# skhu101/SHERF

Measured on AMD Instinct MI355X. Metric: rendered rays/sec at 512x512x64 samples (ImportanceRenderer.forward), higher is better.
Workload: dtype f16 MFMA (fp16 operands rounded to nearest, one product, fp32 accumulate), fp32 elsewhere

## Files before the change

sherf_amd/csrc/gather.hip:

```cpp
#include "common.h"

#ifndef SHERF_GATHER_BRANCHLESS
#define SHERF_GATHER_BRANCHLESS 0
#endif

namespace {

struct Levels { sherf_vox_level l[3]; };

__device__ __forceinline__ void axpy4(float4& a, float w, const float4 v) {
    a.x += w * v.x; a.y += w * v.y; a.z += w * v.z; a.w += w * v.w;
}

__device__ __forceinline__ float clampf(float x, float lo, float hi) { return fminf(fmaxf(x, lo), hi); }

typedef _Float16 h16x4 __attribute__((ext_vector_type(4)));
template <bool HT>
__device__ __forceinline__ float4 ldq(const void* __restrict__ base, size_t idx) {
    if constexpr (HT) {
        const h16x4 v = reinterpret_cast<const h16x4*>(base)[idx];
        return make_float4((float)v[0], (float)v[1], (float)v[2], (float)v[3]);
    } else {
        return reinterpret_cast<const float4*>(base)[idx];
    }
// ... 115 lines not shown
                    }
                    if constexpr (BL) {
#pragma unroll
                    for (int t = 0; t < 8; ++t) {
                        const float w = rec[t].x ? ((t & 1) ? fx : 1.f - fx) * (((t >> 1) & 1) ? fy : 1.f - fy) * ((t >> 2) ? fz : 1.f - fz) : 0.f;
                        const size_t r = (size_t)(rec[t].x ? rec[t].y : 0u) * 24;
                        axpy4(acc[0], w, ldq<HT>(lev.rows, r + l));
                        axpy4(acc[1], w, ldq<HT>(lev.rows, r + 8 + l));
                        axpy4(acc[2], w, ldq<HT>(lev.rows, r + 16 + l));
                    }
                    } else {
#pragma unroll
                    for (int t = 0; t < 8; ++t) {
                        if (rec[t].x) {
                            const float w = ((t & 1) ? fx : 1.f - fx) * (((t >> 1) & 1) ? fy : 1.f - fy) * ((t >> 2) ? fz : 1.f - fz);
                            const size_t r = (size_t)rec[t].y * 24;
                            axpy4(acc[0], w, ldq<HT>(lev.rows, r + l));
                            axpy4(acc[1], w, ldq<HT>(lev.rows, r + 8 + l));
                            axpy4(acc[2], w, ldq<HT>(lev.rows, r + 16 + l));
                        }
                    }
                    }
                }
            }
        } else {
            acc[0] = acc[1] = acc[2] = make_float4(0.f, 0.f, 0.f, 0.f);
            if (mode != 2) {
                extras[(tile * 12 + l) * 32 + j] = 0.f;
                if (l < 4) extras[(tile * 12 + 8 + l) * 32 + j] = 0.f;
            }
        }
        if (mode == 2) {
            if (c < nv)
#pragma unroll
                for (int s = 0; s < 3; ++s) {
                    float4 t = tokens[((tile * 3 + s) * 8 + l) * 32 + j];
                    t.x += acc[s].x; t.y += acc[s].y; t.z += acc[s].z; t.w += acc[s].w;
                    tokens[((tile * 3 + s) * 8 + l) * 32 + j] = t;
                }
            continue;
        }
#pragma unroll
        for (int s = 0; s < 3; ++s) tokens[((tile * 3 + s) * 8 + l) * 32 + j] = acc[s];
    }
}

typedef _Float16 h16x8 __attribute__((ext_vector_type(8)));
constexpr int kPeStride = 120;
__device__ __forceinline__ int64_t banded_first_pair(int b, int g, int64_t n_pairs, int dbg) {
    const bool banded = !(dbg & 1024) && g % 8 == 0;
    if (!banded) return b;
    const int64_t per_xcd = (n_pairs + 7) / 8;
    return (int64_t)(b / 8) < per_xcd ? (int64_t)(b % 8) * per_xcd + b / 8 : n_pairs;
}
struct f8 { float4 a, b; };
__device__ __forceinline__ void axpy8(f8& acc, float w, const void* __restrict__ base, uint32_t idx8) {
    const h16x8 v = *reinterpret_cast<const h16x8*>(static_cast<const char*>(base) + (size_t)(idx8 * 16u));
    acc.a.x += w * (float)v[0]; acc.a.y += w * (float)v[1]; acc.a.z += w * (float)v[2]; acc.a.w += w * (float)v[3];
    acc.b.x += w * (float)v[4]; acc.b.y += w * (float)v[5]; acc.b.z += w * (float)v[6]; acc.b.w += w * (float)v[7];
}

template <bool STAGE, bool PE = false, bool PF = false>
__global__ void __launch_bounds__(256) gather_tokens_h8_kernel(const int32_t* __restrict__ counters, const float* __restrict__ geom,
                                                               const void* __restrict__ planes_f, int P, const void* __restrict__ feat_f,
                                                               int Hf, int Wf, const float4* __restrict__ img4, int H, int W, Levels lv,
                                                               const float4* __restrict__ tok_bias, const float* __restrict__ bounds,
                                                               const float* __restrict__ vox_min, int3 vox_sh, int64_t capacity,
                                                               float4* __restrict__ tokens, float* __restrict__ extras, int dbg, int mode,
                                                               uint4* __restrict__ pefrag) {
    const int64_t nv = min((int64_t)counters[0], capacity);
    int64_t t_lo, t_hi;
    sherf_part_range((nv + 31) / 32, (mode >> 8) & 255, (mode >> 16) & 255, t_lo, t_hi);
    mode &= 255;
    const int64_t n_tiles = t_hi - t_lo, n_pairs = (n_tiles + 1) / 2;
    extern __shared__ __attribute__((aligned(16))) uint2 s_wp[];
    int s_n1 = 0;
    if constexpr (STAGE) {
        const int n1 = (lv.l[1].D * lv.l[1].H * lv.l[1].W + 31) / 32, n2 = (lv.l[2].D * lv.l[2].H * lv.l[2].W + 31) / 32;
        s_n1 = n1;
        if ((banded_first_pair(blockIdx.x, gridDim.x, n_pairs, dbg)) < n_pairs && mode != 1) {
            for (int i = threadIdx.x; i < n1; i += 256) s_wp[i] = reinterpret_cast<const uint2*>(lv.l[1].wp)[i];
            for (int i = threadIdx.x; i < n2; i += 256) s_wp[n1 + i] = reinterpret_cast<const uint2*>(lv.l[2].wp)[i];
        }
        __syncthreads();
    }
    const int l = threadIdx.x & 3;
    const int js = threadIdx.x >> 2;
    const bool banded = !(dbg & 1024) && gridDim.x % 8 == 0;
    const int64_t per_xcd = (n_pairs + 7) / 8, slots = gridDim.x / 8;
    for (int64_t it = banded ? blockIdx.x / 8 : blockIdx.x; it < (banded ? per_xcd : n_pairs); it += banded ? slots : gridDim.x) {
        const int64_t pair = banded ? (int64_t)(blockIdx.x % 8) * per_xcd + it : it;
        if (pair >= n_pairs) break;
        int64_t tile = pair * 2 + (js >> 5);
        const int j = js & 31;
        if (tile >= n_tiles) continue;
        tile += t_lo;
        const int64_t c = tile * 32 + j;
        f8 acc[3];
        if (mode == 2) { for (int s_ = 0; s_ < 3; ++s_) acc[s_].a = acc[s_].b = make_float4(0.f, 0.f, 0.f, 0.f); }
        else { for (int s_ = 0; s_ < 3; ++s_) { acc[s_].a = tok_bias[8 * s_ + 2 * l]; acc[s_].b = tok_bias[8 * s_ + 2 * l + 1]; } }
        float4 rgb = make_float4(0.f, 0.f, 0.f, 0.f);
        const bool valid = c < nv;
        float xv[3] = {0.f, 0.f, 0.f};
        if (valid) {
            const float* gm = geom + c * 8;
            const float xc[3] = {gm[0], gm[1], gm[2]};
            xv[0] = xc[0]; xv[1] = xc[1]; xv[2] = xc[2];
            if (mode != 2) {
                if (l < 3) { extras[(tile * 12 + 2 * l) * 32 + j] = gm[2 * l]; extras[(tile * 12 + 2 * l + 1) * 32 + j] = gm[2 * l + 1]; }
            }
            float n[3];
#pragma unroll
            for (int a = 0; a < 3; ++a) n[a] = 2.f * (xc[a] - bounds[a]) / (bounds[3 + a] - bounds[a]) - 1.f;
#pragma unroll
            for (int p = 0; p < 3; ++p) {
                if ((dbg & 8) || mode == 2) break;
                const float ga = p == 2 ? n[2] : n[0];
                const float gb = p == 1 ? n[2] : n[1];
                float px = clampf(((ga + 1.f) * P - 1.f) * 0.5f, -2.f, (float)P + 1.f);
                float py = clampf(((gb + 1.f) * P - 1.f) * 0.5f, -2.f, (float)P + 1.f);
                float x0 = floorf(px), y0 = floorf(py), fx = px - x0, fy = py - y0;
                int xi = (int)x0, yi = (int)y0;
#pragma unroll
                for (int dy = 0; dy < 2; ++dy)
#pragma unroll
                    for (int dx = 0; dx < 2; ++dx) {
                        int xx = xi + dx, yy = yi + dy;
                        if (xx >= 0 && xx < P && yy >= 0 && yy < P)
                            axpy8(acc[p], (dx ? fx : 1.f - fx) * (dy ? fy : 1.f - fy), planes_f, (uint32_t)(((p * P + yy) * P + xx) * 4 + l));
                    }
            }
            if (!(dbg & 16) && mode != 2) {
                float gx = 2.0f * gm[6] / (float)W - 1.0f, gy = 2.0f * gm[7] / (float)H - 1.0f;
                float px = clampf((gx + 1.f) * 0.5f * (Wf - 1), -2.f, (float)Wf + 1.f);
                float py = clampf((gy + 1.f) * 0.5f * (Hf - 1), -2.f, (float)Hf + 1.f);
                float x0 = floorf(px), y0 = floorf(py), fx = px - x0, fy = py - y0;
                int xi = (int)x0, yi = (int)y0;
#pragma unroll
                for (int dy = 0; dy < 2; ++dy)
#pragma unroll
                    for (int dx = 0; dx < 2; ++dx) {
                        int xx = xi + dx, yy = yi + dy;
                        if (xx >= 0 && xx < Wf && yy >= 0 && yy < Hf) {
                            const float w = (dx ? fx : 1.f - fx) * (dy ? fy : 1.f - fy);
                            const uint32_t t = (uint32_t)((yy * Wf + xx) * 8);
                            axpy8(acc[0], w, feat_f, t + l);
                            axpy8(acc[1], w, feat_f, t + 4 + l);
                        }
                    }
                px = clampf((gx + 1.f) * 0.5f * (W - 1), -2.f, (float)W + 1.f);
                py = clampf((gy + 1.f) * 0.5f * (H - 1), -2.f, (float)H + 1.f);
                x0 = floorf(px); y0 = floorf(py); fx = px - x0; fy = py - y0;
                xi = (int)x0; yi = (int)y0;
#pragma unroll
                for (int dy = 0; dy < 2; ++dy)
#pragma unroll
                    for (int dx = 0; dx < 2; ++dx) {
                        int xx = xi + dx, yy = yi + dy;
                        if (xx >= 0 && xx < W && yy >= 0 && yy < H) axpy4(rgb, (dx ? fx : 1.f - fx) * (dy ? fy : 1.f - fy), img4[(size_t)yy * W + xx]);
                    }
            }
            if (mode != 2) {
                if (l == 3) { extras[(tile * 12 + 6) * 32 + j] = rgb.x; extras[(tile * 12 + 7) * 32 + j] = rgb.y; }
                extras[(tile * 12 + 8 + l) * 32 + j] = (l == 0) ? rgb.z : 0.f;
            }
        } else {
            for (int s_ = 0; s_ < 3; ++s_) acc[s_].a = acc[s_].b = make_float4(0.f, 0.f, 0.f, 0.f);
            if (mode != 2) {
                if (l < 3) { extras[(tile * 12 + 2 * l) * 32 + j] = 0.f; extras[(tile * 12 + 2 * l + 1) * 32 + j] = 0.f; }
                if (l == 3) { extras[(tile * 12 + 6) * 32 + j] = 0.f; extras[(tile * 12 + 7) * 32 + j] = 0.f; }
                extras[(tile * 12 + 8 + l) * 32 + j] = 0.f;
            }
        }
        if (!(dbg & 4) && mode != 1) {
            const float gz = ((xv[2] - vox_min[2]) / 0.005f) / (float)vox_sh.x * 2.f - 1.f;
            const float gy = ((xv[1] - vox_min[1]) / 0.005f) / (float)vox_sh.y * 2.f - 1.f;
            const float gx = ((xv[0] - vox_min[0]) / 0.005f) / (float)vox_sh.z * 2.f - 1.f;
            const int quad0 = (threadIdx.x & 63) & ~3;
#pragma unroll 1
            for (int L = 0; L < 3; ++L) {
                const sherf_vox_level& lev = lv.l[L];
                float px = clampf((gx + 1.f) * 0.5f * (lev.W - 1), -2.f, (float)lev.W + 1.f);
                float py = clampf((gy + 1.f) * 0.5f * (lev.H - 1), -2.f, (float)lev.H + 1.f);
                float pz = clampf((gz + 1.f) * 0.5f * (lev.D - 1), -2.f, (float)lev.D + 1.f);
                float x0 = floorf(px), y0 = floorf(py), z0 = floorf(pz);
                float fx = px - x0, fy = py - y0, fz = pz - z0;
                int xi = (int)x0, yi = (int)y0, zi = (int)z0;
                int mine[2];
#pragma unroll
                for (int u = 0; u < 2; ++u) {
                    const int xx = xi + u, yy = yi + (l & 1), zz = zi + (l >> 1);
                    const bool inb = valid && xx >= 0 && xx < lev.W && yy >= 0 && yy < lev.H && zz >= 0 && zz < lev.D;
                    const int key = inb ? (zz * lev.H + yy) * lev.W + xx : 0;
                    uint2 rr;
                    if (STAGE && L > 0) rr = s_wp[(L == 2 ? s_n1 : 0) + (key >> 5)];
                    else rr = reinterpret_cast<const uint2*>(lev.wp)[key >> 5];
                    const uint32_t bit = 1u << (key & 31);
                    mine[u] = (inb && (rr.x & bit)) ? (int)(rr.y + __popc(rr.x & (bit - 1u))) : -1;
                }
                if constexpr (PF) {
                    int rows8[8];
#pragma unroll
                    for (int t = 0; t < 8; ++t) rows8[t] = __shfl(mine[t & 1], quad0 | (t >> 1));
                    h16x8 buf[2][3];
                    const char* rb = reinterpret_cast<const char*>(lev.rows);
                    auto request = [&](int t, h16x8 (&b)[3]) {
                        const uint32_t r = ((uint32_t)max(rows8[t], 0) * 12u + l) * 16u;
                        b[0] = *reinterpret_cast<const h16x8*>(rb + (size_t)r);
                        b[1] = *reinterpret_cast<const h16x8*>(rb + (size_t)(r + 64u));
                        b[2] = *reinterpret_cast<const h16x8*>(rb + (size_t)(r + 128u));
                    };
                    request(0, buf[0]);
#pragma unroll
                    for (int t = 0; t < 8; ++t) {
                        if (t < 7) request(t + 1, buf[(t + 1) & 1]);
                        const float w0 = ((t & 1) ? fx : 1.f - fx) * (((t >> 1) & 1) ? fy : 1.f - fy) * ((t >> 2) ? fz : 1.f - fz);
                        const float w = rows8[t] >= 0 ? w0 : 0.f;
#pragma unroll
                        for (int s_ = 0; s_ < 3; ++s_) {
                            const h16x8 v = buf[t & 1][s_];
                            acc[s_].a.x += w * (float)v[0]; acc[s_].a.y += w * (float)v[1]; acc[s_].a.z += w * (float)v[2]; acc[s_].a.w += w * (float)v[3];
                            acc[s_].b.x += w * (float)v[4]; acc[s_].b.y += w * (float)v[5]; acc[s_].b.z += w * (float)v[6]; acc[s_].b.w += w * (float)v[7];
                        }
                        __builtin_amdgcn_sched_barrier(0);
                    }
                } else {
#pragma unroll
                for (int t = 0; t < 8; ++t) {
                    const int row = __shfl(mine[t & 1], quad0 | (t >> 1));
                    if (row >= 0) {
                        const float w = ((t & 1) ? fx : 1.f - fx) * (((t >> 1) & 1) ? fy : 1.f - fy) * ((t >> 2) ? fz : 1.f - fz);
                        const uint32_t r = (uint32_t)row * 12u;
                        axpy8(acc[0], w, lev.rows, r + l);
                        axpy8(acc[1], w, lev.rows, r + 4 + l);
                        axpy8(acc[2], w, lev.rows, r + 8 + l);
                    }
                }
                }
            }
        }
        if (mode == 2) {
            if (c < nv)
#pragma unroll
                for (int s_ = 0; s_ < 3; ++s_) {
                    float4* ta = tokens + ((tile * 3 + s_) * 8 + 2 * l) * 32 + j;
                    float4 t0 = ta[0], t1 = ta[32];
                    t0.x += acc[s_].a.x; t0.y += acc[s_].a.y; t0.z += acc[s_].a.z; t0.w += acc[s_].a.w;
                    t1.x += acc[s_].b.x; t1.y += acc[s_].b.y; t1.z += acc[s_].b.z; t1.w += acc[s_].b.w;
                    ta[0] = t0; ta[32] = t1;
                }
            continue;
        }
#pragma unroll
        for (int s_ = 0; s_ < 3; ++s_) {
            tokens[((tile * 3 + s_) * 8 + 2 * l) * 32 + j] = acc[s_].a;
            tokens[((tile * 3 + s_) * 8 + 2 * l + 1) * 32 + j] = acc[s_].b;
        }
        if constexpr (PE) {
            __shared__ __attribute__((aligned(16))) _Float16 s_pe[64 * kPeStride];
            _Float16* sp = s_pe + js * kPeStride;
            float v3[3] = {0.f, 0.f, 0.f};
            if (valid) { const float* gm = geom + c * 8; v3[0] = gm[3]; v3[1] = gm[4]; v3[2] = gm[5]; }
            if (l < 3) {
                const float u6 = l == 0 ? xv[0] : l == 1 ? xv[1] : xv[2];
                const float u4 = l == 0 ? v3[0] : l == 1 ? v3[1] : v3[2];
                const float u5 = l == 0 ? rgb.x : l == 1 ? rgb.y : rgb.z;
                sp[l] = (_Float16)u6; sp[48 + l] = (_Float16)u4; sp[80 + l] = (_Float16)u5;
#pragma unroll
                for (int q = 0; q < 6; ++q) {
                    float sn, cs;
                    sherf_sincos_exact_phase(u6 * (float)(1 << q), &sn, &cs);
                    sp[3 + 6 * q + l] = (_Float16)sn; sp[6 + 6 * q + l] = (_Float16)cs;
                }
#pragma unroll
                for (int q = 0; q < 4; ++q) {
                    float sn, cs;
                    sherf_sincos_exact_phase(u4 * (float)(1 << q), &sn, &cs);
                    sp[48 + 3 + 6 * q + l] = (_Float16)sn; sp[48 + 6 + 6 * q + l] = (_Float16)cs;
                }
#pragma unroll
                for (int q = 0; q < 5; ++q) {
                    float sn, cs;
                    sherf_sincos_exact_phase(u5 * (float)(1 << q), &sn, &cs);
                    sp[80 + 3 + 6 * q + l] = (_Float16)sn;
                    if (q < 4 || l < 2) sp[80 + 6 + 6 * q + l] = (_Float16)cs;
                }
            } else {
                sp[39] = (_Float16)0.f;
                *reinterpret_cast<uint4*>(sp + 40) = make_uint4(0u, 0u, 0u, 0u);
                sp[48 + 27] = (_Float16)0.f;
                *reinterpret_cast<uint2*>(sp + 48 + 28) = make_uint2(0u, 0u);
            }
            __builtin_amdgcn_wave_barrier();
#pragma unroll
            for (int i = 0; i < 4; ++i) {
                const int g = l + 4 * i;
                if (g < 14) pefrag[((tile * 7 + (g >> 1)) * 2 + (g & 1)) * 32 + j] = *reinterpret_cast<const uint4*>(sp + 8 * g);
            }
            __builtin_amdgcn_wave_barrier();
        }
    }
}

__global__ void __launch_bounds__(256, 4) gather_tokens_h16_kernel(const int32_t* __restrict__ counters, const float* __restrict__ geom,
                                                                const void* __restrict__ planes_f, int P, const void* __restrict__ feat_f,
                                                                int Hf, int Wf, const float4* __restrict__ img4, int H, int W, Levels lv,
                                                                const float4* __restrict__ tok_bias, const float* __restrict__ bounds,
                                                                const float* __restrict__ vox_min, int3 vox_sh, int64_t capacity,
                                                                float4* __restrict__ tokens, float* __restrict__ extras, int dbg) {
    const int64_t nv = min((int64_t)counters[0], capacity);
    const int64_t n_tiles = (nv + 31) / 32, n_groups = (n_tiles + 3) / 4;
    const int l = threadIdx.x & 1;
    const int js = threadIdx.x >> 1;
    const bool banded = !(dbg & 1024) && gridDim.x % 8 == 0;
    const int64_t per_xcd = (n_groups + 7) / 8, slots = gridDim.x / 8;
    for (int64_t it = banded ? blockIdx.x / 8 : blockIdx.x; it < (banded ? per_xcd : n_groups); it += banded ? slots : gridDim.x) {
        const int64_t group = banded ? (int64_t)(blockIdx.x % 8) * per_xcd + it : it;
        if (group >= n_groups) break;
        const int64_t tile = group * 4 + (js >> 5);
        const int j = js & 31;
        if (tile >= n_tiles) continue;
        const int64_t c = tile * 32 + j;
        f8 acc[3][2];
#pragma unroll
        for (int s_ = 0; s_ < 3; ++s_)
#pragma unroll
            for (int o = 0; o < 2; ++o) { acc[s_][o].a = tok_bias[8 * s_ + 2 * (2 * l + o)]; acc[s_][o].b = tok_bias[8 * s_ + 2 * (2 * l + o) + 1]; }
        float4 rgb = make_float4(0.f, 0.f, 0.f, 0.f);
        const bool valid = c < nv;
        float xv[3] = {0.f, 0.f, 0.f};
        if (valid) {
            const float* gm = geom + c * 8;
            const float xc[3] = {gm[0], gm[1], gm[2]};
            xv[0] = xc[0]; xv[1] = xc[1]; xv[2] = xc[2];
            if (l == 0) {
#pragma unroll
                for (int r = 0; r < 6; ++r) extras[(tile * 12 + r) * 32 + j] = gm[r];
            }
            float n[3];
#pragma unroll
            for (int a = 0; a < 3; ++a) n[a] = 2.f * (xc[a] - bounds[a]) / (bounds[3 + a] - bounds[a]) - 1.f;
#pragma unroll
            for (int p = 0; p < 3; ++p) {
                if (dbg & 8) break;
                const float ga = p == 2 ? n[2] : n[0];
                const float gb = p == 1 ? n[2] : n[1];
                float px = clampf(((ga + 1.f) * P - 1.f) * 0.5f, -2.f, (float)P + 1.f);
                float py = clampf(((gb + 1.f) * P - 1.f) * 0.5f, -2.f, (float)P + 1.f);
                float x0 = floorf(px), y0 = floorf(py), fx = px - x0, fy = py - y0;
                int xi = (int)x0, yi = (int)y0;
#pragma unroll
                for (int dy = 0; dy < 2; ++dy)
#pragma unroll
                    for (int dx = 0; dx < 2; ++dx) {
                        int xx = xi + dx, yy = yi + dy;
                        if (xx >= 0 && xx < P && yy >= 0 && yy < P) {
                            const float w = (dx ? fx : 1.f - fx) * (dy ? fy : 1.f - fy);
                            const uint32_t t = (uint32_t)(((p * P + yy) * P + xx) * 4 + 2 * l);
                            axpy8(acc[p][0], w, planes_f, t);
                            axpy8(acc[p][1], w, planes_f, t + 1);
                        }
                    }
            }
            if (!(dbg & 16)) {
                float gx = 2.0f * gm[6] / (float)W - 1.0f, gy = 2.0f * gm[7] / (float)H - 1.0f;
                float px = clampf((gx + 1.f) * 0.5f * (Wf - 1), -2.f, (float)Wf + 1.f);
                float py = clampf((gy + 1.f) * 0.5f * (Hf - 1), -2.f, (float)Hf + 1.f);
                float x0 = floorf(px), y0 = floorf(py), fx = px - x0, fy = py - y0;
                int xi = (int)x0, yi = (int)y0;
#pragma unroll
                for (int dy = 0; dy < 2; ++dy)
#pragma unroll
                    for (int dx = 0; dx < 2; ++dx) {
                        int xx = xi + dx, yy = yi + dy;
                        if (xx >= 0 && xx < Wf && yy >= 0 && yy < Hf) {
                            const float w = (dx ? fx : 1.f - fx) * (dy ? fy : 1.f - fy);
                            const uint32_t t = (uint32_t)((yy * Wf + xx) * 8 + 2 * l);
                            axpy8(acc[0][0], w, feat_f, t);
                            axpy8(acc[0][1], w, feat_f, t + 1);
                            axpy8(acc[1][0], w, feat_f, t + 4);
                            axpy8(acc[1][1], w, feat_f, t + 5);
                        }
                    }
                px = clampf((gx + 1.f) * 0.5f * (W - 1), -2.f, (float)W + 1.f);
                py = clampf((gy + 1.f) * 0.5f * (H - 1), -2.f, (float)H + 1.f);
                x0 = floorf(px); y0 = floorf(py); fx = px - x0; fy = py - y0;
                xi = (int)x0; yi = (int)y0;
#pragma unroll
                for (int dy = 0; dy < 2; ++dy)
#pragma unroll
                    for (int dx = 0; dx < 2; ++dx) {
                        int xx = xi + dx, yy = yi + dy;
                        if (xx >= 0 && xx < W && yy >= 0 && yy < H) axpy4(rgb, (dx ? fx : 1.f - fx) * (dy ? fy : 1.f - fy), img4[(size_t)yy * W + xx]);
                    }
            }
            if (l == 1) {
                extras[(tile * 12 + 6) * 32 + j] = rgb.x; extras[(tile * 12 + 7) * 32 + j] = rgb.y; extras[(tile * 12 + 8) * 32 + j] = rgb.z;
#pragma unroll
                for (int r = 9; r < 12; ++r) extras[(tile * 12 + r) * 32 + j] = 0.f;
            }
        } else {
#pragma unroll
            for (int s_ = 0; s_ < 3; ++s_) acc[s_][0].a = acc[s_][0].b = acc[s_][1].a = acc[s_][1].b = make_float4(0.f, 0.f, 0.f, 0.f);
#pragma unroll
            for (int r = 0; r < 6; ++r) extras[(tile * 12 + 6 * l + r) * 32 + j] = 0.f;
        }
        if (!(dbg & 4)) {
            const float gz = ((xv[2] - vox_min[2]) / 0.005f) / (float)vox_sh.x * 2.f - 1.f;
            const float gy = ((xv[1] - vox_min[1]) / 0.005f) / (float)vox_sh.y * 2.f - 1.f;
            const float gx = ((xv[0] - vox_min[0]) / 0.005f) / (float)vox_sh.z * 2.f - 1.f;
            const int pair0 = (threadIdx.x & 63) & ~1;
#pragma unroll 1
            for (int L = 0; L < 3; ++L) {
                const sherf_vox_level& lev = lv.l[L];
                float px = clampf((gx + 1.f) * 0.5f * (lev.W - 1), -2.f, (float)lev.W + 1.f);
                float py = clampf((gy + 1.f) * 0.5f * (lev.H - 1), -2.f, (float)lev.H + 1.f);
                float pz = clampf((gz + 1.f) * 0.5f * (lev.D - 1), -2.f, (float)lev.D + 1.f);
                float x0 = floorf(px), y0 = floorf(py), z0 = floorf(pz);
                float fx = px - x0, fy = py - y0, fz = pz - z0;
                int xi = (int)x0, yi = (int)y0, zi = (int)z0;
                int mine[4];
#pragma unroll
                for (int u = 0; u < 4; ++u) {
                    const int xx = xi + (u & 1), yy = yi + (u >> 1), zz = zi + l;
                    const bool inb = valid && xx >= 0 && xx < lev.W && yy >= 0 && yy < lev.H && zz >= 0 && zz < lev.D;
                    const int key = inb ? (zz * lev.H + yy) * lev.W + xx : 0;
                    const uint2 rr = reinterpret_cast<const uint2*>(lev.wp)[key >> 5];
                    const uint32_t bit = 1u << (key & 31);
                    mine[u] = (inb && (rr.x & bit)) ? (int)(rr.y + __popc(rr.x & (bit - 1u))) : -1;
                }
#pragma unroll
                for (int t = 0; t < 8; ++t) {
                    const int row = __shfl(mine[t & 3], pair0 | (t >> 2));
                    if (row >= 0) {
                        const float w = ((t & 1) ? fx : 1.f - fx) * (((t >> 1) & 1) ? fy : 1.f - fy) * ((t >> 2) ? fz : 1.f - fz);
                        const uint32_t r = (uint32_t)row * 12u + 2u * l;
#pragma unroll
                        for (int s_ = 0; s_ < 3; ++s_) {
                            axpy8(acc[s_][0], w, lev.rows, r + 4 * s_);
                            axpy8(acc[s_][1], w, lev.rows, r + 4 * s_ + 1);
                        }
                    }
                }
            }
        }
#pragma unroll
        for (int s_ = 0; s_ < 3; ++s_)
#pragma unroll
            for (int o = 0; o < 2; ++o) {
                tokens[((tile * 3 + s_) * 8 + 4 * l + 2 * o) * 32 + j] = acc[s_][o].a;
                tokens[((tile * 3 + s_) * 8 + 4 * l + 2 * o + 1) * 32 + j] = acc[s_][o].b;
            }
    }
}

__device__ __forceinline__ void scatter4(float4* dst, float w, const float4 d) {
    float* p = reinterpret_cast<float*>(dst);
    unsafeAtomicAdd(p + 0, w * d.x); unsafeAtomicAdd(p + 1, w * d.y); unsafeAtomicAdd(p + 2, w * d.z); unsafeAtomicAdd(p + 3, w * d.w);
}

struct LevelsBwd { sherf_vox_level l[3]; float* d_rows[3]; };

__global__ void __launch_bounds__(256) gather_tokens_bwd_kernel(const int32_t* __restrict__ counters, const float* __restrict__ geom,
                                                                const float4* __restrict__ d_tokens, int P, int Hf, int Wf, int H, int W,
                                                                LevelsBwd lv, const float* __restrict__ bounds,
                                                                const float* __restrict__ vox_min, int3 vox_sh, int64_t capacity,
                                                                float4* __restrict__ d_planes_f, float4* __restrict__ d_feat_f,
                                                                float* __restrict__ d_tok_bias) {
    __shared__ float s_bias[3][32];
    const int64_t nv = min((int64_t)counters[0], capacity);
    const int64_t n_tiles = (nv + 31) / 32;
    const int l = threadIdx.x & 7, j = threadIdx.x >> 3;
    float4 bsum[3] = {make_float4(0.f, 0.f, 0.f, 0.f), make_float4(0.f, 0.f, 0.f, 0.f), make_float4(0.f, 0.f, 0.f, 0.f)};
    for (int64_t tile = blockIdx.x; tile < n_tiles; tile += gridDim.x) {
        const int64_t c = tile * 32 + j;
        if (c >= nv) continue;
        float4 d[3];
#pragma unroll
        for (int s = 0; s < 3; ++s) {
            d[s] = d_tokens[((tile * 3 + s) * 8 + l) * 32 + j];
            bsum[s].x += d[s].x; bsum[s].y += d[s].y; bsum[s].z += d[s].z; bsum[s].w += d[s].w;
        }
        const float* gm = geom + c * 8;
        const float xc[3] = {gm[0], gm[1], gm[2]};
        float n[3];
#pragma unroll
        for (int a = 0; a < 3; ++a) n[a] = 2.f * (xc[a] - bounds[a]) / (bounds[3 + a] - bounds[a]) - 1.f;
#pragma unroll
        for (int p = 0; p < 3; ++p) {
            const float ga = p == 2 ? n[2] : n[0];
            const float gb = p == 1 ? n[2] : n[1];
            float px = clampf(((ga + 1.f) * P - 1.f) * 0.5f, -2.f, (float)P + 1.f);
            float py = clampf(((gb + 1.f) * P - 1.f) * 0.5f, -2.f, (float)P + 1.f);
            float x0 = floorf(px), y0 = floorf(py), fx = px - x0, fy = py - y0;
            int xi = (int)x0, yi = (int)y0;
#pragma unroll
            for (int dy = 0; dy < 2; ++dy)
#pragma unroll
                for (int dx = 0; dx < 2; ++dx) {
                    int xx = xi + dx, yy = yi + dy;
                    if (xx >= 0 && xx < P && yy >= 0 && yy < P)
                        scatter4(d_planes_f + ((size_t)(p * P + yy) * P + xx) * 8 + l, (dx ? fx : 1.f - fx) * (dy ? fy : 1.f - fy), d[p]);
                }
        }
        {
            float gx = 2.0f * gm[6] / (float)W - 1.0f, gy = 2.0f * gm[7] / (float)H - 1.0f;
            float px = clampf((gx + 1.f) * 0.5f * (Wf - 1), -2.f, (float)Wf + 1.f);
            float py = clampf((gy + 1.f) * 0.5f * (Hf - 1), -2.f, (float)Hf + 1.f);
            float x0 = floorf(px), y0 = floorf(py), fx = px - x0, fy = py - y0;
            int xi = (int)x0, yi = (int)y0;
#pragma unroll
            for (int dy = 0; dy < 2; ++dy)
#pragma unroll
                for (int dx = 0; dx < 2; ++dx) {
                    int xx = xi + dx, yy = yi + dy;
                    if (xx >= 0 && xx < Wf && yy >= 0 && yy < Hf) {
                        const float w = (dx ? fx : 1.f - fx) * (dy ? fy : 1.f - fy);
                        float4* t = d_feat_f + ((size_t)yy * Wf + xx) * 16;
                        scatter4(t + l, w, d[0]);
                        scatter4(t + 8 + l, w, d[1]);
                    }
                }
        }
        {
            float gz = ((xc[2] - vox_min[2]) / 0.005f) / (float)vox_sh.x * 2.f - 1.f;
            float gy = ((xc[1] - vox_min[1]) / 0.005f) / (float)vox_sh.y * 2.f - 1.f;
            float gx = ((xc[0] - vox_min[0]) / 0.005f) / (float)vox_sh.z * 2.f - 1.f;
#pragma unroll 1
            for (int L = 0; L < 3; ++L) {
                const sherf_vox_level& lev = lv.l[L];
                float px = clampf((gx + 1.f) * 0.5f * (lev.W - 1), -2.f, (float)lev.W + 1.f);
                float py = clampf((gy + 1.f) * 0.5f * (lev.H - 1), -2.f, (float)lev.H + 1.f);
                float pz = clampf((gz + 1.f) * 0.5f * (lev.D - 1), -2.f, (float)lev.D + 1.f);
                float x0 = floorf(px), y0 = floorf(py), z0 = floorf(pz);
                float fx = px - x0, fy = py - y0, fz = pz - z0;
                int xi = (int)x0, yi = (int)y0, zi = (int)z0;
#pragma unroll
                for (int t = 0; t < 8; ++t) {
                    const int xx = xi + (t & 1), yy = yi + ((t >> 1) & 1), zz = zi + (t >> 2);
                    if (!(xx >= 0 && xx < lev.W && yy >= 0 && yy < lev.H && zz >= 0 && zz < lev.D)) continue;
                    const int key = (zz * lev.H + yy) * lev.W + xx;
                    const uint2 rr = reinterpret_cast<const uint2*>(lev.wp)[key >> 5];
                    const uint32_t bit = 1u << (key & 31);
                    if (!(rr.x & bit)) continue;
                    const size_t row = rr.y + __popc(rr.x & (bit - 1u));
                    const float w = ((t & 1) ? fx : 1.f - fx) * (((t >> 1) & 1) ? fy : 1.f - fy) * ((t >> 2) ? fz : 1.f - fz);
                    float4* rp = reinterpret_cast<float4*>(lv.d_rows[L]) + row * 24;
                    scatter4(rp + l, w, d[0]);
                    scatter4(rp + 8 + l, w, d[1]);
                    scatter4(rp + 16 + l, w, d[2]);
                }
            }
        }
    }
    for (int i = threadIdx.x; i < 96; i += 256) (&s_bias[0][0])[i] = 0.f;
    __syncthreads();
#pragma unroll
    for (int s = 0; s < 3; ++s) {
        atomicAdd(&s_bias[s][4 * l + 0], bsum[s].x); atomicAdd(&s_bias[s][4 * l + 1], bsum[s].y);
        atomicAdd(&s_bias[s][4 * l + 2], bsum[s].z); atomicAdd(&s_bias[s][4 * l + 3], bsum[s].w);
    }
    __syncthreads();
    for (int i = threadIdx.x; i < 96; i += 256) unsafeAtomicAdd(d_tok_bias + i, (&s_bias[0][0])[i]);
}


constexpr int kBinNT = 256;

struct VoxTap { int xi, yi, zi; float fx, fy, fz; };

__device__ __forceinline__ void vox_grid_coords(const float* __restrict__ gm, const float* __restrict__ vox_min, int3 vox_sh, float& gx, float& gy, float& gz) {
    gz = ((gm[2] - vox_min[2]) / 0.005f) / (float)vox_sh.x * 2.f - 1.f;
    gy = ((gm[1] - vox_min[1]) / 0.005f) / (float)vox_sh.y * 2.f - 1.f;
    gx = ((gm[0] - vox_min[0]) / 0.005f) / (float)vox_sh.z * 2.f - 1.f;
}

__device__ __forceinline__ VoxTap vox_tap(const sherf_vox_level& lev, float gx, float gy, float gz) {
    const float px = clampf((gx + 1.f) * 0.5f * (lev.W - 1), -2.f, (float)lev.W + 1.f);
    const float py = clampf((gy + 1.f) * 0.5f * (lev.H - 1), -2.f, (float)lev.H + 1.f);
    const float pz = clampf((gz + 1.f) * 0.5f * (lev.D - 1), -2.f, (float)lev.D + 1.f);
    const float x0 = floorf(px), y0 = floorf(py), z0 = floorf(pz);
    return VoxTap{(int)x0, (int)y0, (int)z0, px - x0, py - y0, pz - z0};
}

struct PlaneTap { int xi, yi; float fx, fy; };
__device__ __forceinline__ PlaneTap plane_tap(int p, const float* n, int P) {
    const float ga = p == 2 ? n[2] : n[0], gb = p == 1 ? n[2] : n[1];
    const float px = clampf(((ga + 1.f) * P - 1.f) * 0.5f, -2.f, (float)P + 1.f);
    const float py = clampf(((gb + 1.f) * P - 1.f) * 0.5f, -2.f, (float)P + 1.f);
    const float x0 = floorf(px), y0 = floorf(py);
    return PlaneTap{(int)x0, (int)y0, px - x0, py - y0};
}

struct PixTap { int xi, yi; float fx, fy; };
__device__ __forceinline__ PixTap pix_tap(const float* __restrict__ gm, int W, int H, int Wf, int Hf) {
    const float gx = 2.0f * gm[6] / (float)W - 1.0f, gy = 2.0f * gm[7] / (float)H - 1.0f;
    const float px = clampf((gx + 1.f) * 0.5f * (Wf - 1), -2.f, (float)Wf + 1.f);
    const float py = clampf((gy + 1.f) * 0.5f * (Hf - 1), -2.f, (float)Hf + 1.f);
    const float x0 = floorf(px), y0 = floorf(py);
    return PixTap{(int)x0, (int)y0, px - x0, py - y0};
}

__device__ __forceinline__ int bin_of(const sherf_vox_level& lev, const VoxTap& t) {
    return ((t.zi + 2) * (lev.H + 4) + (t.yi + 2)) * (lev.W + 4) + (t.xi + 2);
}

struct BinWs { int32_t *n_nonempty, *counts, *cursor, *offsets, *nonempty, *bin, *sorted, *blocks; int n_bins; };
__host__ __device__ inline BinWs bin_ws(int32_t* scratch, int n_bins, int64_t cap) {
    BinWs w;
    w.n_nonempty = scratch; w.counts = scratch + 4; w.cursor = w.counts + n_bins; w.offsets = w.cursor + n_bins; w.nonempty = w.offsets + n_bins;
    w.bin = w.nonempty + n_bins; w.sorted = w.bin + cap; w.blocks = w.sorted + cap; w.n_bins = n_bins;
    return w;
}

__global__ void __launch_bounds__(256) bin_count_kernel(const int32_t* __restrict__ counters, const float* __restrict__ geom, sherf_vox_level lev2,
                                                        const float* __restrict__ vox_min, int3 vox_sh, int64_t capacity, BinWs w) {
    const int64_t nv = min((int64_t)counters[0], capacity);
    const int64_t c = (int64_t)blockIdx.x * 256 + threadIdx.x;
    if (c >= nv) return;
    float gx, gy, gz;
    vox_grid_coords(geom + c * 8, vox_min, vox_sh, gx, gy, gz);
    const int b = bin_of(lev2, vox_tap(lev2, gx, gy, gz));
    w.bin[c] = b;
    if (atomicAdd(w.counts + b, 1) == 0) w.nonempty[atomicAdd(w.n_nonempty, 1)] = b;
}

__global__ void __launch_bounds__(1024) bin_scan_kernel(BinWs w) {
    __shared__ int s_tot[1024];
    const int per = (w.n_bins + 1023) / 1024;
    const int b0 = min((int)threadIdx.x * per, w.n_bins), b1 = min(b0 + per, w.n_bins);
    int t = 0;
    for (int b = b0; b < b1; ++b) t += w.counts[b];
    s_tot[threadIdx.x] = t;
    __syncthreads();
    for (int o = 1; o < 1024; o <<= 1) {
        const int v = threadIdx.x >= (unsigned)o ? s_tot[threadIdx.x - o] : 0;
        __syncthreads();
        s_tot[threadIdx.x] += v;
        __syncthreads();
    }
    int run = s_tot[threadIdx.x] - t;
    for (int b = b0; b < b1; ++b) { w.offsets[b] = run; run += w.counts[b]; }
}

__global__ void __launch_bounds__(256) bin_fill_kernel(const int32_t* __restrict__ counters, int64_t capacity, BinWs w) {
    const int64_t nv = min((int64_t)counters[0], capacity);
    const int64_t c = (int64_t)blockIdx.x * 256 + threadIdx.x;
    if (c >= nv) return;
    const int b = w.bin[c];
    w.sorted[w.offsets[b] + atomicAdd(w.cursor + b, 1)] = (int32_t)c;
}

__global__ void __launch_bounds__(kBinNT) gather_tokens_bwd_binned_kernel(const float* __restrict__ geom, const float4* __restrict__ d_tokens, int P, int Hf,
                                                                          int Wf, int H, int W, LevelsBwd lv, const float* __restrict__ bounds,
                                                                          const float* __restrict__ vox_min, int3 vox_sh, BinWs w,
                                                                          float4* __restrict__ d_planes_f, float4* __restrict__ d_feat_f,
                                                                          float* __restrict__ d_tok_bias, int dbg) {
    const bool do_pix = !(dbg & 16384), do_vox = !(dbg & 32768), do_pl = !(dbg & 65536), reg2 = !(dbg & 8192);
    __shared__ float s_bias[96];
    const int tid = threadIdx.x, lane = tid & 63, wv = tid >> 6, half = lane >> 5, c31 = lane & 31;
    const int n_list = *w.n_nonempty;
    const sherf_vox_level levs[3] = {lv.l[0], lv.l[1], lv.l[2]};
    float* const drows[3] = {lv.d_rows[0], lv.d_rows[1], lv.d_rows[2]};
    const float* dt = reinterpret_cast<const float*>(d_tokens);
    float* const dpl = reinterpret_cast<float*>(d_planes_f);
    float* const dfm = reinterpret_cast<float*>(d_feat_f);
    float bs0 = 0.f, bs1 = 0.f;
    for (int bi = blockIdx.x; bi < n_list; bi += gridDim.x) {
        const int b = w.nonempty[bi], cnt = w.counts[b], start = w.offsets[b];
        float a2[8], b2[4];
#pragma unroll
        for (int k = 0; k < 8; ++k) a2[k] = 0.f;
#pragma unroll
        for (int k = 0; k < 4; ++k) b2[k] = 0.f;
        int row2 = -1;
        for (int base = wv * 64; base < cnt; base += (kBinNT / 64) * 64) {
            const bool live = base + lane < cnt;
            const int cs = live ? w.sorted[start + base + lane] : 0;
            int tv[24], tp[12], tf[4];
            float wvx[24], wpl[12], wfm[4];
            {
                const float* gm = geom + (int64_t)cs * 8;
                float n[3];
#pragma unroll
                for (int a = 0; a < 3; ++a) n[a] = 2.f * (gm[a] - bounds[a]) / (bounds[3 + a] - bounds[a]) - 1.f;
#pragma unroll
                for (int p = 0; p < 3; ++p) {
                    const PlaneTap t = plane_tap(p, n, P);
#pragma unroll
                    for (int k = 0; k < 4; ++k) {
                        const int xx = t.xi + (k & 1), yy = t.yi + (k >> 1);
                        tp[4 * p + k] = (live && do_pl && xx >= 0 && xx < P && yy >= 0 && yy < P) ? (p * P + yy) * P + xx : -1;
                        wpl[4 * p + k] = ((k & 1) ? t.fx : 1.f - t.fx) * ((k >> 1) ? t.fy : 1.f - t.fy);
                    }
                }
                const PixTap t = pix_tap(gm, W, H, Wf, Hf);
#pragma unroll
                for (int k = 0; k < 4; ++k) {
                    const int xx = t.xi + (k & 1), yy = t.yi + (k >> 1);
                    tf[k] = (live && do_pix && xx >= 0 && xx < Wf && yy >= 0 && yy < Hf) ? yy * Wf + xx : -1;
                    wfm[k] = ((k & 1) ? t.fx : 1.f - t.fx) * ((k >> 1) ? t.fy : 1.f - t.fy);
                }
                float gx, gy, gz;
                vox_grid_coords(gm, vox_min, vox_sh, gx, gy, gz);
#pragma unroll
                for (int L = 0; L < 3; ++L) {
                    const sherf_vox_level lev = levs[L];
                    const VoxTap vt = vox_tap(lev, gx, gy, gz);
#pragma unroll
                    for (int k = 0; k < 8; ++k) {
                        const int xx = vt.xi + (k & 1), yy = vt.yi + ((k >> 1) & 1), zz = vt.zi + (k >> 2);
                        wvx[8 * L + k] = (live && do_vox) ? ((k & 1) ? vt.fx : 1.f - vt.fx) * (((k >> 1) & 1) ? vt.fy : 1.f - vt.fy) * ((k >> 2) ? vt.fz : 1.f - vt.fz) : 0.f;
                        int tg = -1;
                        if (live && do_vox && xx >= 0 && xx < lev.W && yy >= 0 && yy < lev.H && zz >= 0 && zz < lev.D) {
                            const int key = (zz * lev.H + yy) * lev.W + xx;
                            const uint2 rr = reinterpret_cast<const uint2*>(lev.wp)[key >> 5];
                            const uint32_t bit = 1u << (key & 31);
                            if (rr.x & bit) tg = (int)(rr.y + __popc(rr.x & (bit - 1u)));
                        }
                        tv[8 * L + k] = tg;
                    }
                }
            }
            if (base == wv * 64) {
#pragma unroll
                for (int k = 0; k < 8; ++k) {
                    const int r = __builtin_amdgcn_readlane(tv[16 + k], 0);
                    if (lane == k) row2 = r;
                }
            }
            const int nact = min(64, cnt - base);
            for (int sidx = 0; sidx < nact; ++sidx) {
                const int c = __builtin_amdgcn_readlane(cs, sidx);
                const int64_t tile = c >> 5;
                const int j = c & 31;
                const int64_t dbase = (((tile * 3) * 8 + (c31 >> 2)) * 32 + j) * 4 + (c31 & 3);
                const float dp0 = dt[dbase], dp1 = dt[dbase + 1024], d1 = dt[dbase + 2048];
                const float d0 = half ? dp1 : dp0;
                bs0 += d0; bs1 += half ? 0.f : d1;
#define SHERF_RL(v) __builtin_amdgcn_readlane((v), sidx)
#define SHERF_RLF(v) __int_as_float(__builtin_amdgcn_readlane(__float_as_int(v), sidx))
#pragma unroll
                for (int p = 0; p < 3; ++p) {
                    const float dpv = p == 0 ? dp0 : (p == 1 ? dp1 : d1);
#pragma unroll
                    for (int dy = 0; dy < 2; ++dy) {
// ... 478 lines not shown
```

Measured before the change: 163.4 million.

## Prefetch voxel occupancy words for all levels before plane sampling

```diff
diff --git a/sherf_amd/csrc/gather.hip b/sherf_amd/csrc/gather.hip
--- a/sherf_amd/csrc/gather.hip
+++ b/sherf_amd/csrc/gather.hip
@@ -441,11 +441,18 @@
     }
 }
 
+__device__ __forceinline__ int in_loop(int v) {
+#if defined(__HIP_DEVICE_COMPILE__)
+    asm volatile("" : "+s"(v));
+#endif
+    return v;
+}
+
 __global__ void __launch_bounds__(256, 4) gather_tokens_h16_kernel(const int32_t* __restrict__ counters, const float* __restrict__ geom,
-                                                                const void* __restrict__ planes_f, int P, const void* __restrict__ feat_f,
-                                                                int Hf, int Wf, const float4* __restrict__ img4, int H, int W, Levels lv,
+                                                                const void* __restrict__ planes_f, int P_, const void* __restrict__ feat_f,
+                                                                int Hf_, int Wf_, const float4* __restrict__ img4, int H_, int W_, Levels lv,
                                                                 const float4* __restrict__ tok_bias, const float* __restrict__ bounds,
-                                                                const float* __restrict__ vox_min, int3 vox_sh, int64_t capacity,
+                                                                const float* __restrict__ vox_min, int3 vox_sh_, int64_t capacity,
                                                                 float4* __restrict__ tokens, float* __restrict__ extras, int dbg) {
     const int64_t nv = min((int64_t)counters[0], capacity);
     const int64_t n_tiles = (nv + 31) / 32, n_groups = (n_tiles + 3) / 4;
@@ -460,18 +467,53 @@
         const int j = js & 31;
         if (tile >= n_tiles) continue;
         const int64_t c = tile * 32 + j;
+        const int P = in_loop(P_), Hf = in_loop(Hf_), Wf = in_loop(Wf_), H = in_loop(H_), W = in_loop(W_);
+        const int3 vox_sh = make_int3(in_loop(vox_sh_.x), in_loop(vox_sh_.y), in_loop(vox_sh_.z));
+        const bool valid = c < nv;
+        float xv[3] = {0.f, 0.f, 0.f};
+        if (valid) { const float* gm = geom + c * 8; xv[0] = gm[0]; xv[1] = gm[1]; xv[2] = gm[2]; }
+        const float gz = ((xv[2] - vox_min[2]) / 0.005f) / (float)vox_sh.x * 2.f - 1.f;
+        const float gy = ((xv[1] - vox_min[1]) / 0.005f) / (float)vox_sh.y * 2.f - 1.f;
+        const float gx = ((xv[0] - vox_min[0]) / 0.005f) / (float)vox_sh.z * 2.f - 1.f;
+        int mine[3][4];
+        uint2 rec[3][4];
+        uint32_t rbit[3][4];
+        if (!(dbg & 4)) {
+#pragma unroll
+            for (int L = 0; L < 3; ++L) {
+                const sherf_vox_level& lev = lv.l[L];
+                const int lW = in_loop(lev.W), lH = in_loop(lev.H), lD = in_loop(lev.D);
+                const float px = clampf((gx + 1.f) * 0.5f * (lW - 1), -2.f, (float)lW + 1.f);
+                const float py = clampf((gy + 1.f) * 0.5f * (lH - 1), -2.f, (float)lH + 1.f);
+                const float pz = clampf((gz + 1.f) * 0.5f * (lD - 1), -2.f, (float)lD + 1.f);
+                const int xi = (int)floorf(px), yi = (int)floorf(py), zi = (int)floorf(pz);
+#pragma unroll
+                for (int u = 0; u < 4; ++u) {
+                    const int xx = xi + (u & 1), yy = yi + (u >> 1), zz = zi + l;
+                    const bool inb = valid && xx >= 0 && xx < lev.W && yy >= 0 && yy < lev.H && zz >= 0 && zz < lev.D;
+                    const int key = inb ? (zz * lev.H + yy) * lev.W + xx : 0;
+                    rec[L][u] = reinterpret_cast<const uint2*>(lev.wp)[key >> 5];
+                    rbit[L][u] = inb ? 1u << (key & 31) : 0u;
+                }
+            }
+#pragma unroll
+            for (int L = 0; L < 3; ++L)
+#pragma unroll
+                for (int u = 0; u < 4; ++u) {
+                    const uint2 rr = rec[L][u];
+                    const uint32_t bit = rbit[L][u];
+                    mine[L][u] = (rr.x & bit) ? (int)(rr.y + __popc(rr.x & (bit - 1u))) : -1;
+                }
+        }
         f8 acc[3][2];
 #pragma unroll
         for (int s_ = 0; s_ < 3; ++s_)
 #pragma unroll
             for (int o = 0; o < 2; ++o) { acc[s_][o].a = tok_bias[8 * s_ + 2 * (2 * l + o)]; acc[s_][o].b = tok_bias[8 * s_ + 2 * (2 * l + o) + 1]; }
         float4 rgb = make_float4(0.f, 0.f, 0.f, 0.f);
-        const bool valid = c < nv;
-        float xv[3] = {0.f, 0.f, 0.f};
         if (valid) {
             const float* gm = geom + c * 8;
-            const float xc[3] = {gm[0], gm[1], gm[2]};
-            xv[0] = xc[0]; xv[1] = xc[1]; xv[2] = xc[2];
+            const float xc[3] = {xv[0], xv[1], xv[2]};
             if (l == 0) {
 #pragma unroll
                 for (int r = 0; r < 6; ++r) extras[(tile * 12 + r) * 32 + j] = gm[r];
@@ -545,9 +587,6 @@
             for (int r = 0; r < 6; ++r) extras[(tile * 12 + 6 * l + r) * 32 + j] = 0.f;
         }
         if (!(dbg & 4)) {
-            const float gz = ((xv[2] - vox_min[2]) / 0.005f) / (float)vox_sh.x * 2.f - 1.f;
-            const float gy = ((xv[1] - vox_min[1]) / 0.005f) / (float)vox_sh.y * 2.f - 1.f;
-            const float gx = ((xv[0] - vox_min[0]) / 0.005f) / (float)vox_sh.z * 2.f - 1.f;
             const int pair0 = (threadIdx.x & 63) & ~1;
 #pragma unroll 1
             for (int L = 0; L < 3; ++L) {
@@ -557,20 +596,9 @@
                 float pz = clampf((gz + 1.f) * 0.5f * (lev.D - 1), -2.f, (float)lev.D + 1.f);
                 float x0 = floorf(px), y0 = floorf(py), z0 = floorf(pz);
                 float fx = px - x0, fy = py - y0, fz = pz - z0;
-                int xi = (int)x0, yi = (int)y0, zi = (int)z0;
-                int mine[4];
-#pragma unroll
-                for (int u = 0; u < 4; ++u) {
-                    const int xx = xi + (u & 1), yy = yi + (u >> 1), zz = zi + l;
-                    const bool inb = valid && xx >= 0 && xx < lev.W && yy >= 0 && yy < lev.H && zz >= 0 && zz < lev.D;
-                    const int key = inb ? (zz * lev.H + yy) * lev.W + xx : 0;
-                    const uint2 rr = reinterpret_cast<const uint2*>(lev.wp)[key >> 5];
-                    const uint32_t bit = 1u << (key & 31);
-                    mine[u] = (inb && (rr.x & bit)) ? (int)(rr.y + __popc(rr.x & (bit - 1u))) : -1;
-                }
 #pragma unroll
                 for (int t = 0; t < 8; ++t) {
-                    const int row = __shfl(mine[t & 3], pair0 | (t >> 2));
+                    const int row = __shfl(mine[0][t & 3], pair0 | (t >> 2));
                     if (row >= 0) {
                         const float w = ((t & 1) ? fx : 1.f - fx) * (((t >> 1) & 1) ? fy : 1.f - fy) * ((t >> 2) ? fz : 1.f - fz);
                         const uint32_t r = (uint32_t)row * 12u + 2u * l;
@@ -581,6 +609,8 @@
                         }
                     }
                 }
+#pragma unroll
+                for (int u = 0; u < 4; ++u) { mine[0][u] = mine[1][u]; mine[1][u] = mine[2][u]; }
             }
         }
 #pragma unroll
```

Result: no change. 164.5 million, median of 6 (+0.6%).
